# renmengye/rec-attend-public

Hardware: AMD Instinct MI355X
Metric: instance-timesteps/sec, full_model forward 512x512 T=16 (whole job; pipelined throughput: 8 batches in flight per GPU, fill and drain of the pipeline inside the timed region; config.lone_batch_* = one sync-bracketed forward) (higher is better)
Workload: dtype f32; 1 GPU; cfg2: CVPPP-arch full_model eval forward, 512x512, T=16, B=8 per GPU, y_out+s_out; arch=cvppp, H=512, W=512, T=16, batch_per_gpu=8, global_batch=8, parallelism=batch-sharded x1, no collective, ranks_in_communicator=1, hip_graph=True, tile_tickets=False, batches_in_flight=8, pipeline_slots=4, batches_per_launch=2, input=resident in HBM, output=left in HBM

## Files before the change

include/recattend.h:

```cpp
#ifndef RECATTEND_H_
#define RECATTEND_H_

#include <stddef.h>
#include <stdint.h>

#ifdef __cplusplus
extern "C" {
#endif

#define RA_E_INVALID (-1)
#define RA_E_SHAPE (-2)
#define RA_E_WORKSPACE (-3)
#define RA_E_HUNG_BFS (-12)
#define RA_E_HUNG_PATH (-13)
#define RA_E_HUNG_FLOW (-14)
#define RA_E_HUNG_EQUALIZE (-15)

#define RA_ABI_VERSION 114
int ra_version(void);
const char *ra_last_error_string(void);

int ra_debug_poison_lds(void *stream);
int ra_debug_park_xcd(int xcd, int n_wg, int lds_bytes, int millis, int *resident, void *stream);

// ... 227 lines not shown
int ra_extract_conv0_f32(const float *img, int Ci, int chan0, const float *canvas, int canvas_chan,
                         const float *attn_rec, int B, int H, int W, int Fh, int Fw, int use_gamma, float *patch,
                         const float *w0, const float *scale, const float *shift, int Cout, int relu, float *y0,
                         void *stream);
#define RA_PASTE_Y_PREFILLED 1
#define RA_PASTE_CANVAS_FLOORED 2
int ra_paste_direct_f32(const float *patch, int Cp, int pc, const float *attn, int B, int H, int W,
                        int Fh, int Fw, float beta, int disable_overwrite, float *canvas, float *img,
                        int Ci, int canvas_chan, float *y_out, size_t y_stride_b, int flags,
                        void *stream);
int ra_paste_score_direct_f32(const float *patch, int Cp, int pc, const float *attn, int B, int H,
                              int W, int Fh, int Fw, float beta, int disable_overwrite,
                              float *canvas, float *y_out, size_t y_stride_b, int flags,
                              const float *h, int K0, const float *core, int K1, const float *w,
                              const float *bias, float *s_out, size_t s_stride_b, void *stream);

#define RA_RESAMPLE_READ 0
#define RA_RESAMPLE_WRITE 1
#define RA_RESAMPLE_BOX 2
int ra_ctrl_train_supported(int G, int Cf, int hid, int iters, int nout);
size_t ra_ctrl_train_save_floats(int G, int Cf, int hid, int iters);
int ra_ctrl_train_fwd_f32(int B, int G, int Cf, int hid, int iters, int nout, const float *feat, const float *Wg,
                          const float *bg, const float *W0, const float *b0, const float *W1, const float *b1,
                          const float *Wc, const float *bc, float *h_last, float *co, float *save, void *stream);
int ra_ctrl_train_bwd_f32(int B, int G, int Cf, int hid, int iters, int nout, const float *feat, const float *Wg,
                          const float *W0, const float *W1, const float *Wc, const float *save, const float *dh_last,
                          const float *dco, float *dfeat, float *dpre, float *dz1, float *dlog, void *stream);
int ra_ctrl_train_supported_n(int G, int Cf, int hid, int iters, int nout, int n_glimpse, int n_ctrl, int mlp_dim);
size_t ra_ctrl_train_save_floats_n(int G, int Cf, int hid, int iters, int n_glimpse);
int ra_ctrl_train_fwd_n_f32(int B, int G, int Cf, int hid, int iters, int nout, int n_glimpse, int n_ctrl, int mlp_dim,
// ... 12 lines not shown
                        int Fw, const float *scale, int scale_stride, const float *div, int div_stride, float *ws,
                        size_t ws_floats, float *out, void *stream);
int ra_attn_box_direct_f32(const float *attn, int B, int H, int W, int Fh, int Fw, float beta,
                           float *box_out, size_t stride_b, void *stream);

int ra_extract_patch_dense_f32(const float *x, const float *f_y, const float *f_x, int B, int H,
                               int W, int D, int FH, int FW, float *out, void *stream);

int ra_dense_f32(const float *x0, int K0, const float *x1, int K1, const float *W, const float *b,
                 int B, int N, int act, float *out, size_t out_stride_b, void *stream);

int ra_pack_input_f32(const float *x, int D, const float *d_in, int Dd, const float *y_in, int Dy,
                      int B, int H, int W, int Cp, float *packed, void *stream);
int ra_pack_input_plane_f32(const float *x, int D, const float *d_in, int Dd, const float *y_in, int Dy,
                            int B, int H, int W, int Cp, float *packed, float *canvas_plane, void *stream);
int ra_canvas_max_f32(float *img, int Ci, int canvas_chan, const float *ysel, const float *noise,
                      int B, int H, int W, void *stream);

int ra_affine_act_f32(const float *x, const float *scale, const float *shift, size_t npix, int C,
                      int relu, float *y, void *stream);
int ra_max_pool_f32(const float *x, int B, int H, int W, int C, int ratio, float *y, void *stream);

enum {
  RA_STAT_LOSS = 0, RA_STAT_BOX_LOSS, RA_STAT_SEGM_LOSS, RA_STAT_CONF_LOSS, RA_STAT_IOU_SOFT,
  RA_STAT_IOU_SOFT_BOX, RA_STAT_WT_COV_SOFT, RA_STAT_UNWT_COV_SOFT, RA_STAT_IOU_HARD,
  RA_STAT_WT_COV_HARD, RA_STAT_UNWT_COV_HARD, RA_STAT_DICE, RA_STAT_COUNT_ACC, RA_STAT_DIC,
  RA_STAT_DIC_ABS, RA_STAT_COUNT
};
size_t ra_pair_stats_workspace_floats(int B, int HW);
int ra_pair_stats_f32(const float *a, const float *b, int B, int N, int M, int HW, float *ws,
// ... 320 lines not shown
```

rec-attend-public_amd/csrc/ra_attn.hip:

```cpp
#include "ra_common.h"

namespace ra {
namespace attn {

typedef float f32x4 __attribute__((ext_vector_type(4)));

__device__ inline float tap_mu(float ctr, float size, int F, int j) {
  return ctr + (size + 1.0f) / (float)F * ((float)j - ((float)F - 1.0f) / 2.0f);
}
__device__ inline float gauss(float l, float mu, float var) {
  const float d = l - mu;
  return (1.0f / sqrtf(var) / sqrtf(2.0f * 3.14159265358979323846f)) * expf(-0.5f * d * d / var);
}

__global__ void gaussian_filter_kernel(const float *center, const float *size, const float *lg_var,
                                       int B, int L, int F, float *out) {
  const size_t n = (size_t)B * L * F;
  for (size_t e = blockIdx.x * (size_t)blockDim.x + threadIdx.x; e < n;
       e += (size_t)gridDim.x * blockDim.x) {
    const int f = e % F;
    const int l = (e / F) % L;
    const int b = e / ((size_t)F * L);
    out[e] = gauss((float)l, tap_mu(center[b], size[b], F, f), expf(lg_var[b]));
  }
// ... 25 lines not shown
      __syncthreads();
      if (o < nout) {
        int wlo = (c0 - d + D - 1) / D;
        if (wlo < 0) wlo = 0;
        for (int w = wlo; w < W; ++w) {
          const int idx = w * D + d - c0;
          if (idx >= cn) break;
          acc += tbuf[idx] * fxb[(size_t)w * FW + fw];
        }
      }
    }
    if (o < nout) out[(((size_t)b * FH + fh) * FW + fw) * D + d] = acc;
  }
}

__global__ void pack_input_kernel(const float *x, int D, const float *d_in, int Dd, const float *y_in,
                                  int Dy, size_t npix, int Cp, float *packed, float *plane) {
  const int C4 = Cp >> 2;
  const size_t n = npix * C4;
  typedef float f32x4p __attribute__((ext_vector_type(4)));
  for (size_t e = blockIdx.x * (size_t)blockDim.x + threadIdx.x; e < n; e += (size_t)gridDim.x * blockDim.x) {
    const size_t p = e / C4;
    const int q = (int)(e - p * C4);
    if (plane && q == 0) plane[p] = 0.0f;
    f32x4p v;
#pragma unroll
    for (int j = 0; j < 4; ++j) {
      const int c = 4 * q + j;
      float val = 0.0f;
      if (c < D) val = x[p * D + c];
      else if (c > D && c <= D + Dd) val = d_in[p * Dd + (c - D - 1)];
      else if (c > D + Dd && c <= D + Dd + Dy) val = y_in[p * Dy + (c - D - 1 - Dd)];
      v[j] = val;
    }
    reinterpret_cast<f32x4p *>(packed)[e] = v;
  }
}

__global__ void canvas_max_kernel(float *img, int Ci, int canvas_chan, const float *ysel,
                                  const float *noise, size_t npix) {
  for (size_t p = blockIdx.x * (size_t)blockDim.x + threadIdx.x; p < npix;
       p += (size_t)gridDim.x * blockDim.x) {
    float v = ysel[p];
    if (noise) v = v - v * noise[p];
    float *c = img + p * Ci + canvas_chan;
    *c = fmaxf(v, *c);
  }
}

__global__ void affine_act_kernel(const float *x, const float *scale, const float *shift, size_t n,
// ... 63 lines not shown
}

extern "C" int ra_pack_input_plane_f32(const float *x, int D, const float *d_in, int Dd, const float *y_in,
                                       int Dy, int B, int H, int W, int Cp, float *packed, float *canvas_plane,
                                       void *stream) {
  if (!x || !packed || B <= 0 || H <= 0 || W <= 0 || D <= 0 || (Dd > 0 && !d_in) || (Dy > 0 && !y_in))
    return fail(RA_E_INVALID, "ra_pack_input_f32: bad argument");
  if (Cp % 4 || D + 1 + Dd + Dy > Cp || (reinterpret_cast<uintptr_t>(packed) & 15))
    return fail(RA_E_SHAPE, "ra_pack_input_f32: Cp %d (a multiple of 4 holding D + 1 + Dd + Dy channels), packed 16-byte aligned", Cp);
  const size_t npix = (size_t)B * H * W;
  hipLaunchKernelGGL(attn::pack_input_kernel, dim3(attn::grid_for(npix * (size_t)(Cp / 4), 256)), dim3(256), 0,
                     as_stream(stream), x, D, d_in, Dd, y_in, Dy, npix, Cp, packed, canvas_plane);
  return launch_status("ra_pack_input_f32");
}

extern "C" int ra_canvas_max_f32(float *img, int Ci, int canvas_chan, const float *ysel,
                                 const float *noise, int B, int H, int W, void *stream) {
  if (!img || !ysel || B <= 0 || H <= 0 || W <= 0 || canvas_chan < 0 || canvas_chan >= Ci)
    return fail(RA_E_INVALID, "ra_canvas_max_f32: bad argument");
  const size_t npix = (size_t)B * H * W;
  hipLaunchKernelGGL(attn::canvas_max_kernel, dim3(attn::grid_for(npix, 256)), dim3(256), 0,
                     as_stream(stream), img, Ci, canvas_chan, ysel, noise, npix);
  return launch_status("ra_canvas_max_f32");
}

extern "C" int ra_affine_act_f32(const float *x, const float *scale, const float *shift, size_t npix,
                                 int C, int relu, float *y, void *stream) {
  if (!x || !scale || !shift || !y || C <= 0) return fail(RA_E_INVALID, "ra_affine_act_f32: bad argument");
  if (npix == 0) return 0;
  const size_t n = npix * C;
// ... 16 lines not shown
```

rec-attend-public_amd/csrc/ra_attn_axis.h:

```cpp
#pragma once
#include "ra_common.h"

namespace ra {
namespace attnd {

typedef float f32x4 __attribute__((ext_vector_type(4)));
constexpr float kBandLog = 30.0f;
constexpr float kInvSqrt2Pi = 0.3989422804014327f;

struct Axis {
  float ctr, step, inv_step, half, inv2var, norm, R;
  int L, F;
  __device__ inline float mu(int j) const { return ctr + step * ((float)j - half); }
  __device__ inline float w(float l, int j) const {
    const float d = l - mu(j);
    return norm * __expf(-d * d * inv2var);
  }
  __device__ inline void band(int j, int &lo, int &hi) const {
    const float m = mu(j);
    float a = ceilf(m - R), c = floorf(m + R) + 1.0f;
    a = fminf(fmaxf(a, 0.0f), (float)L);
    c = fminf(fmaxf(c, 0.0f), (float)L);
    if (!(a == a) || !(c == c)) {
      a = 0.0f;
// ... 31 lines not shown
__device__ inline Axis make_axis(const float *rec, int axis, int L, int F) {
  Axis A;
  const float var = __expf(rec[4 + axis]);
  A.ctr = rec[0 + axis];
  A.step = (rec[2 + axis] + 1.0f) / (float)F;
  A.inv_step = __builtin_amdgcn_rcpf(A.step);
  A.half = ((float)F - 1.0f) / 2.0f;
  A.inv2var = 0.5f * __builtin_amdgcn_rcpf(var);
  A.norm = kInvSqrt2Pi * __builtin_amdgcn_rsqf(var);
  A.R = __builtin_amdgcn_sqrtf(2.0f * kBandLog * var);
  A.L = L;
  A.F = F;
  return A;
}

__device__ inline float readlane_f(float v, int l) {
  return __builtin_bit_cast(float, __builtin_amdgcn_readlane(__builtin_bit_cast(int, v), l));
}

}
}
```

rec-attend-public_amd/csrc/ra_attn_direct.hip:

```cpp
#include <cstdlib>

#include "ra_attn_parts.h"
#include "ra_common.h"

namespace ra {
namespace attnd {

#ifdef RA_PROBE
__device__ long long *ra_probe_buf;
#define RA_PROBE_AT(k)                                                                              \
  do {                                                                                              \
    if (threadIdx.x == 0)                                                                           \
      ra_probe_buf[(size_t)(blockIdx.x + gridDim.x * (blockIdx.y + gridDim.y * blockIdx.z)) * 8 + (k)] = wall_clock64(); \
  } while (0)
#else
#define RA_PROBE_AT(k)
#endif

struct Conv0Args {
  const float *w, *scale, *shift;
  int Cout, relu;
  float *y0;
};

// ... 481 lines not shown
    }
#pragma unroll
    for (int r = 0; r < RB; ++r) {
      if (!((live_mask >> r) & 1)) continue;
      const float cv = (MODE == 0) ? Cs[r * W + w] : 0.0f;
      float v = fast_sigmoid(acc[r] + beta);
      v -= dis * v * cv;
      __builtin_amdgcn_raw_buffer_store_b32(__builtin_bit_cast(unsigned, v), rsY, w * 4, r * W * 4, 0);
      if (MODE == 0)
        __builtin_amdgcn_raw_buffer_store_b32(__builtin_bit_cast(unsigned, fmaxf(cv, v)), rsV, w * 4, r * W * 4, 0);
    }
  }
  RA_PROBE_AT(4);
}

}
}

using namespace ra;

namespace {
struct PastePlan {
  int kernel, rows, grid_x, threads;
  size_t lds;
};
PastePlan choose_paste(int mode, int H, int W, int Fh, int Fw, int Cp, int pc, bool has_canvas, bool has_img, size_t y_stride_b,
                       bool aligned16, attnd::PasteGeo pg) {
  const int rb = pg.rows == 8 ? 8 : 4;
  const bool win_ok = W % 4 == 0 && Fw <= 64 && rb * W <= 4096 && (y_stride_b & 3) == 0 && aligned16 &&
                      (size_t)H * W * 4 < 0x7fffffffu && Fh * Fw % 4 == 0 && Fh * Fw <= 4 * attnd::kPsQuads * 256 &&
// ... 101 lines not shown
}

extern "C" int ra_paste_score_direct_f32(const float *patch, int Cp, int pc, const float *attn_rec, int B, int H,
                                         int W, int Fh, int Fw, float beta, int disable_overwrite, float *canvas,
                                         float *y_out, size_t y_stride_b, int flags, const float *h, int K0,
                                         const float *core, int K1, const float *w, const float *bias,
                                         float *s_out, size_t s_stride_b, void *stream) {
  if (!patch || !attn_rec || !y_out || !canvas || !h || !w || !s_out || B <= 0 || H <= 0 || W <= 0 || Fh <= 0 ||
      Fw <= 0 || Cp <= 0 || pc < 0 || pc >= Cp || K0 <= 0 || K1 < 0 || (K1 > 0 && !core))
    return fail(RA_E_INVALID, "ra_paste_score_direct_f32: bad argument");
  attnd::ScoreArgs sc{h, core, w, bias, s_out, K0, K1, s_stride_b};
  launch_paste<0>(1, patch, Cp, pc, attn_rec, B, H, W, Fh, Fw, beta, disable_overwrite, canvas, nullptr, 0, -1, y_out,
                  y_stride_b, disable_overwrite ? (flags & ~RA_PASTE_Y_PREFILLED) : flags, sc, stream);
  return launch_status("ra_paste_score_direct_f32");
}
```

rec-attend-public_amd/full_model.py:

```python
import os
import numpy as np
import torch

import modellib
import nnlib as nn
import ra_engine
import ra_ops as ops
from ra_native import RecAttendError


def _get(opt, key, default):
  return opt[key] if key in opt else default


def derive_dims(opt, box_model=False):
  d = {'T': opt['timespan'], 'H': opt['inp_height'], 'W': opt['inp_width'],
       'D': opt['inp_depth'], 'Fh': opt['filter_height'], 'Fw': opt['filter_width']}
  if d['H'] % 4 or d['W'] % 4:
    raise RecAttendError('inp_height / inp_width must be multiples of 4')
  if 'add_d_out' in opt:
    add_d, add_y = bool(opt['add_d_out']), bool(opt['add_y_out'])
  else:
    add_d = add_y = False
  assert (add_d and add_y) or (not add_d and not add_y)
# ... 308 lines not shown
    self.co_resident = int(co_resident or self.streams)
    self.coalesce = int(coalesce)
    self.slots = None
    self.free = list(range(self.depth))
    self.group = []
    self.pending = []

  def _make_slots(self):
    proto = self.model.engine
    self.slots = []
    prios = [int(v) for v in os.environ.get('RA_PIPE_PRIO', '').split(',') if v.strip()]
    streams = [torch.cuda.Stream(priority=prios[k % len(prios)]) if prios else torch.cuda.Stream() for k in range(self.streams)]
    for k in range(self.depth):
      eng = ra_engine.DecodeEngine(proto.d, self.model, box_model=proto.box)
      for flag in ('fuse_pairs', 'fuse_patch_pairs', 'ctrl_split', 'fuse_score',
                   'cache_first', 'fill_cache_inline', 'nsub', 'use_graph', 'use_wino', 'wino_unfuse', 'pair_wino', 'pair_direct16', 'prefill_ride',
                   'fuse_extract_conv0', 'use_split', 'split_first', 'split_patch', 'box_iou_rects', 'ctrl_batch_xcd'):
        setattr(eng, flag, getattr(proto, flag))
      eng.co_resident = self.co_resident
      eng.xcd_slot, eng.xcd_slots = k % self.streams, (self.streams if self.co_resident <= self.streams else 0)
      self.slots.append((eng, streams[k % self.streams]))

  def __len__(self):
    return len(self.pending)

  def parts(self, B):
    return 1 if not self.max_images else max(1, -(-int(B) // int(self.max_images)))

  def _ends_soon(self, remaining):
    return (remaining is not None and self.coalesce > 1 and len(self.group) + 1 + int(remaining) <= self.depth and
            os.environ.get('RA_PIPE_ENDGAME', '0') == '1')
# ... 32 lines not shown
    t = dict(names=names, single=single, feed=feed, to_host=to_host, B=B, launch=None, lo=0, hi=B)
    self.group.append(t)
    self.pending.append(t)
    if len(self.group) >= self.coalesce or ends:
      self._launch_group()

  def _launch_group(self):
    if not self.group:
      return
    members, self.group = self.group, []
    if self.slots is None:
      self._make_slots()
    names, to_host = members[0]['names'], members[0]['to_host']
    feeds = [m['feed'] for m in members]
    as_dev = lambda v: v if isinstance(v, torch.Tensor) else torch.from_numpy(np.ascontiguousarray(v, dtype=np.float32))
    if len(members) == 1:
      feed = feeds[0]
    else:
      feed = {}
      for k in ('x', 'd_in', 'y_in', 'y_gt'):
        if feeds[0].get(k) is not None:
          feed[k] = torch.cat([as_dev(f[k]).to('cuda', non_blocking=True) for f in feeds], dim=0)
      if feeds[0].get('noise') is not None:
        feed['noise'] = torch.cat([as_dev(f['noise']).to('cuda') for f in feeds], dim=1)
    B = sum(m['B'] for m in members)
    nparts = self.parts(B)
    if nparts > len(self.free):
      raise RecAttendError('%d of %d slots busy: collect() a batch before the next submit()' %
                           (self.depth - len(self.free), self.depth))
    bounds = [(B * i) // nparts for i in range(nparts + 1)]
    cut = lambda v, lo, hi: None if v is None else v[lo:hi]
    used, events = [], []
    for lo, hi in zip(bounds[:-1], bounds[1:]):
      k = self.free.pop(0)
      eng, stream = self.slots[k]
      stream.wait_stream(torch.cuda.current_stream())
      noise = feed.get('noise')
      with torch.cuda.stream(stream):
        eng.forward(cut(feed['x'], lo, hi), d_in=cut(feed.get('d_in'), lo, hi), y_in=cut(feed.get('y_in'), lo, hi),
                    y_gt=cut(feed.get('y_gt'), lo, hi) if self.model.box_model else None,
                    noise=None if noise is None else noise[:, lo:hi], want_box='attn_box' in names)
        host = None
        if to_host:
          host = []
          for n in names:
            r = self.model._fetch(n, eng)
# ... 192 lines not shown
```

rec-attend-public_amd/ra_engine.py:

```python
import numpy as np
import math
import os

import torch

import operator

import ra_native as rn
import ra_ops as ops


def _dev(a, device):
  return torch.from_numpy(np.ascontiguousarray(a)).to(device)


def _r4(n):
  return -(-n // 4) * 4


_TENSOR_VERSION = operator.attrgetter('_version')


class DecodeEngine(object):

  def __init__(self, dims, model, box_model=False):
    self.d = dims
    self.model = model
    self.box = box_model
    self._stamp = None
    self._B = None
    self._graphs = {}
    self.fuse_pairs = True
    self.fuse_patch_pairs = False
    self.ctrl_split = True
    self.fuse_score = True
    self.wino_unfuse = False
    self.pair_wino = True
    self.pair_direct16 = os.environ.get('RA_PAIR16', '1') != '0'
    self.use_wino = True
    self.cache_first = True
    self.fill_cache_inline = True
    self.co_resident = 1
    self.tile_tickets = os.environ.get('RA_ENGINE_TICKETS', '0') != '0'
    self.nsub = 0
    self.use_graph = True
    self.prefill_ride = True
    self.use_split = os.environ.get('RA_USE_SPLIT', '1') != '0'
    self.split_first = os.environ.get('RA_SPLIT_FIRST', '1') != '0'
    self.ctrl_batch_xcd = os.environ.get('RA_CTRL_BATCH_XCD', '1') != '0'
    self.xcd_slot, self.xcd_slots = 0, 1
    self.box_iou_rects = os.environ.get('RA_BOX_IOU_RECTS', '1') != '0'
    self.split_patch = os.environ.get('RA_SPLIT_PATCH', 'auto')
    self.fuse_extract_conv0 = os.environ.get('RA_FUSE_EXTRACT_CONV0', '0') == '1'
    self.timing = None

  def _weights_stamp(self):
    m = self.model
    mut = getattr(m, '_mut', None)
    if mut is None:
      return tuple((k, v.data_ptr(), v._version) for k, v in sorted(m.items())
                   if isinstance(v, torch.Tensor) and '_' in k and not k.startswith('__'))
# ... 212 lines not shown
    subs = []
    for k in range(nsub):
      b = {kk: v[k * Bs:(k + 1) * Bs] for kk, v in g.items() if kk != 'noise'}
      b['img'] = f(Bs, H, W, d['C0p'])
      b['canvas'] = f(Bs, H, W)
      hh, ww = H, W
      b['ccnn'] = []
      for i in range(d['ccnn_nlayers']):
        hh, ww = hh // d['ccnn_pool'][i], ww // d['ccnn_pool'][i]
        b['ccnn'].append(f(Bs, hh, ww, d['ccnn_channels'][i + 1]))
      b['tickets'] = ops.tickets_alloc(16 * T, device)
      b['h_last'] = f(T, Bs, d['hid'])
      b['ctrl_out'] = f(T, Bs, 9)
      b['gmaps'] = f(T, Bs, d['iters'], d['G'])
      b['attn'] = f(T, Bs, rn.RA_ATTN_STRIDE)
      st0 = self.plan['ccnn'][0]
      if self.cache_first and st0[0] == 'pair' and d['C0p'] == 4 and self.ksize['ccnn'][:2] == [3, 3] and \
          ops.first_cache_supported(4, d['ccnn_channels'][1], d['ccnn_channels'][2], d['ccnn_pool'][1], H, W):
        b['l0cache'] = ops.first_cache_alloc(Bs, H, W, device)
      form = ops.ctrl_form(self.desc, Bs, self.co_resident) if self.split_ok else None
      if form == 'split':
        b['ctrl_ws'], b['ctrl_status'] = ops.ctrl_split_workspace(self.desc, Bs, device)
      elif form == 'batch':
        b['ctrl_ws'], b['ctrl_status'] = ops.ctrl_batch_workspace(self.desc, Bs, device)
        b['ctrl_batch'] = True
        ng = -(-Bs // ops.ctrl_batch_group(self.desc, Bs))
        if self.ctrl_batch_xcd and self.xcd_slots >= 1 and self.xcd_slots * ng <= int(os.environ.get('RA_CTRL_BATCH_XCD_MAX_TEAMS', '4')):
          b['ctrl_xcd_off'] = (self.xcd_slot % self.xcd_slots) * ng
      if self.box:
        b['noise'] = f(T, Bs, H, W)
# ... 19 lines not shown
    self.glob = g
    self.subs = subs
    self.streams = [torch.cuda.Stream(device=device) for _ in range(nsub)] if nsub > 1 else []
    self._B = (B, nsub)
    self._graphs = {}

  def fetch(self, name):
    if name in self.glob:
      return self.glob[name]
    parts = [sb[name] for sb in self.subs]
    if len(parts) == 1:
      return parts[0]
    dim = 0 if name in ('img', 'canvas') else 1
    return torch.cat(parts, dim=dim)

  def check_status(self, recover=True):
    bad = False
    for sb in self.subs:
      st = sb.get('ctrl_status')
      if st is not None and int(st.item()) != 0:
        st.zero_()
        bad = True
    if not bad:
      return False
    if not recover:
      raise rn.RecAttendError('controller_split: a workgroup timed out waiting for its peers (the launch was '
                              'not fully resident); decode with engine.ctrl_split = False')
    import warnings
    warnings.warn('controller_split: a workgroup timed out waiting for its peers (the launch was not fully resident: is '
                  'something else using this GPU?); the batch is decoded again on the one-workgroup controller, which this '
                  'engine keeps from now on')
    torch.cuda.synchronize()
    keep = {k: self.glob[k].clone() for k in ('x', 'd_in', 'y_in', 'y_gt', 'noise') if k in self.glob}
    want_box = getattr(self, '_last_want_box', False)
    self.ctrl_split = False
    self._stamp = None
    self._B = None
    self._states = {}
    self._graphs = {}
    self.forward(keep['x'], d_in=keep.get('d_in'), y_in=keep.get('y_in'), y_gt=keep.get('y_gt'), noise=keep.get('noise'),
                 want_box=want_box)
    torch.cuda.synchronize()
    return True

  def _mark(self, name):
    if self.timing is not None:
      ev = torch.cuda.Event(enable_timing=True)
      ev.record()
      self.timing.append((name, ev))

  def stage_times_ms(self):
    out = {}
    for (_, e0), (name, e1) in zip(self.timing[:-1], self.timing[1:]):
      tot, n = out.get(name, (0.0, 0))
      out[name] = (tot + e0.elapsed_time(e1), n + 1)
    return out

# ... 3 lines not shown
      return
    main = torch.cuda.current_stream()
    for sb, st in zip(self.subs, self.streams):
      st.wait_stream(main)
      with torch.cuda.stream(st):
        self._launch_sub(sb, want_box)
    for st in self.streams:
      main.wait_stream(st)

  def _launch_sub(self, b, want_box):
    self._launch_pack(b)
    bound = self.tile_tickets and 'tickets' in b and ops.tickets_bind(b['tickets'])
    try:
      for tt in range(self.d['T']):
        self._launch_tail(b, tt, want_box, self._launch_encoder(b, tt))
    finally:
      if bound:
        ops.tickets_unbind()

  def _launch_encoder(self, b, tt):
    fill = b['y_out'] if (tt == 0 and b.pop('_fill_rider', False)) else None
    return self._run_cnn(self.plan['ccnn'], self.W['ccnn'], b['img'], b['ccnn'], tt, 'ctrl_cnn',
                         plane=b['canvas'], cache=b.get('l0cache'), fill=fill)

  def _prefill_rides(self, b):
    st0 = self.plan['ccnn'][0]
    return (self.prefill_ride and 'l0cache' in b and self.fill_cache_inline and st0[0] == 'pair' and
            ops.fill_rider_ok(b['y_out']))

  def _launch_pack(self, b):
    if self._prepacked:
      b['canvas'].zero_()
    else:
      ops.pack_input(b['x'], b.get('d_in'), b.get('y_in'), self.d['C0p'], b['img'],
                     canvas_plane=b['canvas'])
    if not self.box and not self.d['disable_overwrite']:
      if self._prefill_rides(b):
        b['_fill_rider'] = True
      else:
        ops.fill(b['y_out'], 1.0 / (1.0 + math.exp(5.0)))
    if 'l0cache' in b and not self.fill_cache_inline:
      ops.first_cache(b['img'], self.W['ccnn'][0][0], self.d['ccnn_channels'][1], self.d['D'], b['l0cache'])
    self._mark('pack')

  def _launch_tail(self, b, tt, want_box, src):
    d, Wt, T = self.d, self.W, self.d['T']
    H, W, Fh, Fw = d['H'], d['W'], d['Fh'], d['Fw']
    if 'ctrl_ws' in b and b.get('ctrl_batch'):
      ops.controller_batch(self.desc, src, Wt['ctrl_split'], b['h_last'][tt], b['ctrl_out'][tt], b['gmaps'][tt], b['attn'][tt],
                           b['ctrl_ws'], b['ctrl_status'], xcd_offset=b.get('ctrl_xcd_off', -1))
    elif 'ctrl_ws' in b:
      ops.controller_split(
# ... 111 lines not shown
    box = b['box1']
    if self.box_iou_rects and 'gt_params' in b and d['W'] % 4 == 0 and T <= 32:
      iou = ops.box_iou_rects(box.view(box.shape[0], d['H'], d['W']), b['gt_params'])
    else:
      iou = ops.pair_stats(box, b['box_gt'], want=('iou_soft',))['iou_soft']
    ops.greedy_match(iou.view(iou.shape[0], T), out=b['match'])
    ops.weighted_sum(b['match'], b['y_gt'], b['ysel'])
    ops.canvas_max(b['canvas'].view(b['canvas'].shape + (1,)), 0, b['ysel'], b['noise'][tt])
    nsc = d['nsc']
    ops.dense(b['h_last'][tt], self.W['smlp_w'], self.W['smlp_b'],
              'sigmoid' if nsc == 1 else 'softmax', b['s_out'].data_ptr() + tt * nsc * 4,
              T * nsc)
    self._mark('box_step')

  _prepacked = False

  def prestage_slots(self, B):
    if not torch.cuda.is_available():
      raise rn.RecAttendError('the decode loop needs an MI355X (HIP device); no CPU fallback')
    device = torch.device('cuda')
    if self._stamp is None:
      self.prepare(device)
    self.alloc(B, device)
    return self.subs

  def forward(self, x, d_in=None, y_in=None, y_gt=None, noise=None, want_box=False, prepacked=False):
    if not torch.cuda.is_available():
      raise rn.RecAttendError('the decode loop needs an MI355X (HIP device); no CPU fallback')
    self._prepacked = bool(prepacked)
    device = torch.device('cuda')
    as_t = lambda a: (a if isinstance(a, torch.Tensor) else torch.from_numpy(
        np.ascontiguousarray(a, dtype=np.float32))).to(device=device, dtype=torch.float32)
    x = as_t(x)
    B = x.shape[0]
    late_check = self._stamp is not None
    if not late_check:
      self.prepare(device)
    self.alloc(B, device)
    b = self.glob
    b['x'].copy_(x)
    if 'd_in' in b and not prepacked:
      b['d_in'].copy_(as_t(d_in))
    if 'y_in' in b and not prepacked:
      b['y_in'].copy_(as_t(y_in))
    if self.box:
      b['y_gt'].copy_(as_t(y_gt))
      if noise is None:
        b['noise'].uniform_(0.0, 0.3)
      else:
        b['noise'].copy_(as_t(noise).reshape(b['noise'].shape))
      Bs = B // len(self.subs)
      for k, sb in enumerate(self.subs):
        sb['noise'].copy_(b['noise'][:, k * Bs:(k + 1) * Bs])
        sb['gt_params'], sb['box_gt'] = ops.gt_box(sb['y_gt'].contiguous(), float(self.d['attn_box_padding_ratio']), 10.0)
    self._last_want_box = bool(want_box)
    self._launch_forward(want_box)
    if late_check and self._weights_stamp() != self._stamp:
      self.prepare(device)
      self._launch_forward(want_box)
    return self

  def _launch_forward(self, want_box):
    graphable = self.use_graph and self.timing is None
    if not graphable:
      self._launch_all(want_box)
      return self
    key = (bool(want_box), True) if self._prepacked else bool(want_box)
    if self.box:
      for sb in self.subs:
        if 'box_gt_buf' not in sb:
          sb['box_gt_buf'] = torch.empty_like(sb['box_gt'])
          sb['gt_params_buf'] = torch.empty_like(sb['gt_params'])
        sb['box_gt_buf'].copy_(sb['box_gt'])
        sb['box_gt'] = sb['box_gt_buf']
        sb['gt_params_buf'].copy_(sb['gt_params'])
        sb['gt_params'] = sb['gt_params_buf']
    g = self._graphs.get(key)
    if g is None:
      self._launch_all(want_box)
      torch.cuda.synchronize()
      g = torch.cuda.CUDAGraph()
      with rn.quiet_capture(), torch.cuda.graph(g):
        self._launch_all(want_box)
      self._graphs[key] = g
    g.replay()
    return self
```

rec-attend-public_amd/ra_ops.py:

```python
import ctypes as C
import os

import numpy as np
import torch

import ra_native as rn
from ra_native import check, ptr

BN_EPS = 1e-3


def _need_cuda(*ts, f32=True):
  for t in ts:
    if t is not None and not t.is_cuda:
      raise rn.RecAttendError('recattend kernels need CUDA (HIP) tensors; got a CPU tensor. '
                              'There is no CPU fallback.')
    if t is not None and ((f32 and t.dtype != torch.float32) or not t.is_contiguous()):
      raise rn.RecAttendError('recattend kernels need contiguous float32 tensors')


def _np32(a):
  if isinstance(a, torch.Tensor):
    a = a.detach().cpu().numpy()
  return np.ascontiguousarray(a, dtype=np.float32)
# ... 820 lines not shown
PASTE_Y_PREFILLED, PASTE_CANVAS_FLOORED = rn.RA_PASTE_Y_PREFILLED, rn.RA_PASTE_CANVAS_FLOORED


def paste_direct(patch, pc, attn, beta, disable_overwrite, y_out, y_stride_b, H, W, canvas=None,
                 img=None, canvas_chan=-1, flags=0):
  _need_cuda(patch, attn, canvas, img)
  B, Fh, Fw, Cp = patch.shape
  Ci = 0 if img is None else img.shape[3]
  check(rn.lib().ra_paste_direct_f32(ptr(patch), Cp, pc, ptr(attn), B, H, W, Fh, Fw, C.c_float(beta),
                                     int(disable_overwrite), ptr(canvas), ptr(img), Ci,
                                     int(canvas_chan), ptr(y_out), y_stride_b, int(flags),
                                     rn.stream_ptr()),
        'ra_paste_direct_f32')


def paste_score_direct(patch, pc, attn, beta, disable_overwrite, y_out, y_stride_b, H, W, canvas, flags,
                       h, core, w, bias, s_out_ptr, s_stride_b):
  _need_cuda(patch, attn, canvas, h, core, w, bias)
  B, Fh, Fw, Cp = patch.shape
  K1 = 0 if core is None else core.shape[1]
  check(rn.lib().ra_paste_score_direct_f32(ptr(patch), Cp, pc, ptr(attn), B, H, W, Fh, Fw, C.c_float(beta),
                                           int(disable_overwrite), ptr(canvas), ptr(y_out), y_stride_b,
                                           int(flags), ptr(h), h.shape[1], ptr(core), K1, ptr(w), ptr(bias),
                                           ptr(s_out_ptr), s_stride_b, rn.stream_ptr()),
        'ra_paste_score_direct_f32')


def paste_plan(mode, B, H, W, Fh, Fw, Cp=1, pc=0, has_canvas=True, has_img=False, y_stride_b=None, aligned16=True):
  rec = (C.c_int * rn.RA_PASTE_PLAN_INTS)()
  stride = H * W if y_stride_b is None else y_stride_b
# ... 39 lines not shown
  _need_cuda(x0, x1, W, b)
  code = {None: 0, 'relu': 1, 'sigmoid': 2, 'softmax': 3, 'tanh': 4}[act]
  K1 = 0 if x1 is None else x1.shape[1]
  check(rn.lib().ra_dense_f32(ptr(x0), x0.shape[1], ptr(x1), K1, ptr(W), ptr(b), x0.shape[0],
                              W.shape[1], code, ptr(out), out_stride_b, rn.stream_ptr()),
        'ra_dense_f32')


def pack_input(x, d_in, y_in, Cp, packed, canvas_plane=None):
  _need_cuda(x, d_in, y_in, packed, canvas_plane)
  B, H, W, D = x.shape
  Dd = 0 if d_in is None else d_in.shape[3]
  Dy = 0 if y_in is None else y_in.shape[3]
  check(rn.lib().ra_pack_input_plane_f32(ptr(x), D, ptr(d_in), Dd, ptr(y_in), Dy, B, H, W, Cp,
                                         ptr(packed), ptr(canvas_plane), rn.stream_ptr()), 'ra_pack_input_plane_f32')


def canvas_max(img, canvas_chan, ysel, noise):
  _need_cuda(img, ysel, noise)
  B, H, W, Ci = img.shape
  check(rn.lib().ra_canvas_max_f32(ptr(img), Ci, canvas_chan, ptr(ysel), ptr(noise), B, H, W,
                                   rn.stream_ptr()), 'ra_canvas_max_f32')


def gaussian_filter(center, size, lg_var, L, F):
  _need_cuda(center, size, lg_var)
  B = center.shape[0]
  out = torch.empty((B, L, F), dtype=torch.float32, device=center.device)
  check(rn.lib().ra_gaussian_filter_f32(ptr(center), ptr(size), ptr(lg_var), B, L, F, ptr(out),
                                        rn.stream_ptr()), 'ra_gaussian_filter_f32')
# ... 1025 lines not shown
```

Before: 61940 instance-timesteps/s.

## Pack inputs directly from per-batch sources and prefill only attention windows

Adds a multi-source pack kernel so per-batch feeds go straight into the packed image buffer, skipping the torch.cat and the staging copy into glob buffers. Also adds a fill_windows kernel that, once y_out is known clean from a prior run, refills only the rows and columns covered by each step's attention window rather than the whole y_out. A y_clean flag tracks validity and is reset on recovery. The cost is extra bookkeeping and a correctness risk if the flag becomes stale.

```diff
diff --git a/include/recattend.h b/include/recattend.h
--- a/include/recattend.h
+++ b/include/recattend.h
@@ -265,6 +265,8 @@
                               float *canvas, float *y_out, size_t y_stride_b, int flags,
                               const float *h, int K0, const float *core, int K1, const float *w,
                               const float *bias, float *s_out, size_t s_stride_b, void *stream);
+int ra_fill_windows_f32(float *y, size_t y_stride_b, int T, int B, int H, int W, int Fh, int Fw, const float *records,
+                        float value, const int *clean_flag, void *stream);
 
 #define RA_RESAMPLE_READ 0
 #define RA_RESAMPLE_WRITE 1
@@ -307,6 +309,9 @@
                       int B, int H, int W, int Cp, float *packed, void *stream);
 int ra_pack_input_plane_f32(const float *x, int D, const float *d_in, int Dd, const float *y_in, int Dy,
                             int B, int H, int W, int Cp, float *packed, float *canvas_plane, void *stream);
+int ra_pack_input_multi_f32(int nsrc, const float *const *x, const float *const *d_in, const float *const *y_in,
+                            const int *images, int D, int Dd, int Dy, int H, int W, int Cp, float *packed,
+                            float *canvas_plane, void *stream);
 int ra_canvas_max_f32(float *img, int Ci, int canvas_chan, const float *ysel, const float *noise,
                       int B, int H, int W, void *stream);
 
diff --git a/rec-attend-public_amd/csrc/ra_attn.hip b/rec-attend-public_amd/csrc/ra_attn.hip
--- a/rec-attend-public_amd/csrc/ra_attn.hip
+++ b/rec-attend-public_amd/csrc/ra_attn.hip
@@ -1,3 +1,6 @@
+#include <climits>
+#include <cstdint>
+
 #include "ra_common.h"
 
 namespace ra {
@@ -63,26 +66,57 @@
   }
 }
 
+__device__ __forceinline__ f32x4 pack_quad(const float *x, int D, const float *d_in, int Dd, const float *y_in, int Dy,
+                                            size_t p, int q) {
+  f32x4 v;
+#pragma unroll
+  for (int j = 0; j < 4; ++j) {
+    const int c = 4 * q + j;
+    float val = 0.0f;
+    if (c < D) val = x[p * D + c];
+    else if (c > D && c <= D + Dd) val = d_in[p * Dd + (c - D - 1)];
+    else if (c > D + Dd && c <= D + Dd + Dy) val = y_in[p * Dy + (c - D - 1 - Dd)];
+    v[j] = val;
+  }
+  return v;
+}
+
 __global__ void pack_input_kernel(const float *x, int D, const float *d_in, int Dd, const float *y_in,
                                   int Dy, size_t npix, int Cp, float *packed, float *plane) {
   const int C4 = Cp >> 2;
   const size_t n = npix * C4;
-  typedef float f32x4p __attribute__((ext_vector_type(4)));
   for (size_t e = blockIdx.x * (size_t)blockDim.x + threadIdx.x; e < n; e += (size_t)gridDim.x * blockDim.x) {
     const size_t p = e / C4;
     const int q = (int)(e - p * C4);
     if (plane && q == 0) plane[p] = 0.0f;
-    f32x4p v;
+    reinterpret_cast<f32x4 *>(packed)[e] = pack_quad(x, D, d_in, Dd, y_in, Dy, p, q);
+  }
+}
+
+constexpr int kPackSources = 8;
+struct PackSources {
+  const float *x[kPackSources], *d_in[kPackSources], *y_in[kPackSources];
+  size_t first[kPackSources];
+};
+
+__global__ void pack_input_multi_kernel(PackSources S, int D, int Dd, int Dy, size_t npix, int Cp, float *packed, float *plane) {
+  const int C4 = Cp >> 2;
+  const size_t n = npix * C4;
+  for (size_t e = blockIdx.x * (size_t)blockDim.x + threadIdx.x; e < n; e += (size_t)gridDim.x * blockDim.x) {
+    const size_t p = e / C4;
+    const int q = (int)(e - p * C4);
+    if (plane && q == 0) plane[p] = 0.0f;
+    const float *x = S.x[0], *d_in = S.d_in[0], *y_in = S.y_in[0];
+    size_t first = 0;
 #pragma unroll
-    for (int j = 0; j < 4; ++j) {
-      const int c = 4 * q + j;
-      float val = 0.0f;
-      if (c < D) val = x[p * D + c];
-      else if (c > D && c <= D + Dd) val = d_in[p * Dd + (c - D - 1)];
-      else if (c > D + Dd && c <= D + Dd + Dy) val = y_in[p * Dy + (c - D - 1 - Dd)];
-      v[j] = val;
+    for (int s = 1; s < kPackSources; ++s) {
+      const bool in = p >= S.first[s];
+      x = in ? S.x[s] : x;
+      d_in = in ? S.d_in[s] : d_in;
+      y_in = in ? S.y_in[s] : y_in;
+      first = in ? S.first[s] : first;
     }
-    reinterpret_cast<f32x4p *>(packed)[e] = v;
+    reinterpret_cast<f32x4 *>(packed)[e] = pack_quad(x, D, d_in, Dd, y_in, Dy, p - first, q);
   }
 }
 
@@ -176,6 +210,35 @@
   return launch_status("ra_pack_input_f32");
 }
 
+extern "C" int ra_pack_input_multi_f32(int nsrc, const float *const *x, const float *const *d_in, const float *const *y_in,
+                                       const int *images, int D, int Dd, int Dy, int H, int W, int Cp, float *packed,
+                                       float *canvas_plane, void *stream) {
+  if (nsrc < 1 || nsrc > attn::kPackSources || !x || !images || !packed || H <= 0 || W <= 0 || D <= 0 || Dd < 0 || Dy < 0 ||
+      (Dd > 0 && !d_in) || (Dy > 0 && !y_in))
+    return fail(RA_E_INVALID, "ra_pack_input_multi_f32: bad argument (1 .. %d sources)", attn::kPackSources);
+  attn::PackSources S;
+  const size_t hw = (size_t)H * W;
+  size_t B = 0;
+  for (int s = 0; s < attn::kPackSources; ++s) {
+    const bool live = s < nsrc;
+    S.x[s] = live ? x[s] : nullptr;
+    S.d_in[s] = live && d_in ? d_in[s] : nullptr;
+    S.y_in[s] = live && y_in ? y_in[s] : nullptr;
+    S.first[s] = live ? B * hw : SIZE_MAX;
+    if (!live) continue;
+    if (!x[s] || images[s] <= 0 || (S.d_in[s] != nullptr) != (S.d_in[0] != nullptr) || (S.y_in[s] != nullptr) != (S.y_in[0] != nullptr) ||
+        (Dd > 0 && !S.d_in[s]) || (Dy > 0 && !S.y_in[s]))
+      return fail(RA_E_INVALID, "ra_pack_input_multi_f32: source %d: x, d_in (all sources or none), y_in (likewise), images > 0", s);
+    B += (size_t)images[s];
+  }
+  if (Cp % 4 || D + 1 + Dd + Dy > Cp || (reinterpret_cast<uintptr_t>(packed) & 15) || B > (size_t)INT_MAX)
+    return fail(RA_E_SHAPE, "ra_pack_input_multi_f32: Cp %d (a multiple of 4 holding D + 1 + Dd + Dy channels), packed 16-byte aligned", Cp);
+  const size_t npix = B * hw;
+  hipLaunchKernelGGL(attn::pack_input_multi_kernel, dim3(attn::grid_for(npix * (size_t)(Cp / 4), 256)), dim3(256), 0,
+                     as_stream(stream), S, D, Dd, Dy, npix, Cp, packed, canvas_plane);
+  return launch_status("ra_pack_input_multi_f32");
+}
+
 extern "C" int ra_canvas_max_f32(float *img, int Ci, int canvas_chan, const float *ysel,
                                  const float *noise, int B, int H, int W, void *stream) {
   if (!img || !ysel || B <= 0 || H <= 0 || W <= 0 || canvas_chan < 0 || canvas_chan >= Ci)
diff --git a/rec-attend-public_amd/csrc/ra_attn_axis.h b/rec-attend-public_amd/csrc/ra_attn_axis.h
--- a/rec-attend-public_amd/csrc/ra_attn_axis.h
+++ b/rec-attend-public_amd/csrc/ra_attn_axis.h
@@ -69,6 +69,23 @@
   return A;
 }
 
+struct PasteWindow {
+  Axis Ay;
+  int wbeg, wend;
+  __device__ inline bool row(int l) const {
+    int jlo, jhi;
+    Ay.taps(l, jlo, jhi);
+    return jlo < jhi;
+  }
+};
+
+__device__ inline PasteWindow paste_window(const float *rec, int H, int W, int Fh, int Fw) {
+  PasteWindow p;
+  p.Ay = make_axis(rec, 0, H, Fh);
+  make_axis(rec, 1, W, Fw).span4(p.wbeg, p.wend);
+  return p;
+}
+
 __device__ inline float readlane_f(float v, int l) {
   return __builtin_bit_cast(float, __builtin_amdgcn_readlane(__builtin_bit_cast(int, v), l));
 }
diff --git a/rec-attend-public_amd/csrc/ra_attn_direct.hip b/rec-attend-public_amd/csrc/ra_attn_direct.hip
--- a/rec-attend-public_amd/csrc/ra_attn_direct.hip
+++ b/rec-attend-public_amd/csrc/ra_attn_direct.hip
@@ -519,6 +519,30 @@
   RA_PROBE_AT(4);
 }
 
+constexpr int kFillRows = 64;
+__global__ __launch_bounds__(256) void fill_windows_kernel(float *__restrict__ y, size_t y_stride_b, int T, int B, int H, int W,
+                                                            int Fh, int Fw, const float *__restrict__ records, float value,
+                                                            const int *__restrict__ clean, int vec, int chunks) {
+  const int lane = threadIdx.x & 63, wv = __builtin_amdgcn_readfirstlane(threadIdx.x >> 6);
+  const int plane = blockIdx.x / chunks, chunk = blockIdx.x - plane * chunks;
+  const int b = plane / T, t = plane - b * T;
+  const bool whole = *clean == 0;
+  const PasteWindow pw = paste_window(records + ((size_t)t * B + b) * RA_ATTN_STRIDE, H, W, Fh, Fw);
+  const int wbeg = whole ? 0 : pw.wbeg, wend = whole ? W : pw.wend;
+  const f32x4 v4 = f32x4{value, value, value, value};
+  const int l1 = (chunk + 1) * kFillRows < H ? (chunk + 1) * kFillRows : H;
+  float *base = y + (size_t)b * y_stride_b + (size_t)t * H * W;
+  for (int l = chunk * kFillRows + wv; l < l1; l += 4) {
+    if (!whole && !pw.row(l)) continue;
+    float *row = base + (size_t)l * W;
+    if (vec) {
+      for (int w = wbeg + 4 * lane; w < wend; w += 256) *reinterpret_cast<f32x4 *>(row + w) = v4;
+    } else {
+      for (int w = wbeg + lane; w < wend; w += 64) row[w] = value;
+    }
+  }
+}
+
 }
 }
 
@@ -650,3 +674,16 @@
                   y_stride_b, disable_overwrite ? (flags & ~RA_PASTE_Y_PREFILLED) : flags, sc, stream);
   return launch_status("ra_paste_score_direct_f32");
 }
+
+extern "C" int ra_fill_windows_f32(float *y, size_t y_stride_b, int T, int B, int H, int W, int Fh, int Fw, const float *records,
+                                   float value, const int *clean_flag, void *stream) {
+  if (!y || !records || !clean_flag || T <= 0 || B <= 0 || H <= 0 || W <= 0 || Fh <= 0 || Fw <= 0)
+    return fail(RA_E_INVALID, "ra_fill_windows_f32: bad argument");
+  if (y_stride_b < (size_t)T * H * W) return fail(RA_E_SHAPE, "ra_fill_windows_f32: image stride %zu < T H W", y_stride_b);
+  const int vec = W % 4 == 0 && (reinterpret_cast<uintptr_t>(y) & 15) == 0 && (y_stride_b & 3) == 0;
+  const int chunks = ceil_div(H, attnd::kFillRows);
+  if ((size_t)B * T * chunks > 0x7fffffffu) return fail(RA_E_SHAPE, "ra_fill_windows_f32: B T ceil(H / %d) exceeds 2^31", attnd::kFillRows);
+  hipLaunchKernelGGL(attnd::fill_windows_kernel, dim3((unsigned)((size_t)B * T * chunks)), dim3(256), 0, as_stream(stream), y, y_stride_b, T,
+                     B, H, W, Fh, Fw, records, value, clean_flag, vec, chunks);
+  return launch_status("ra_fill_windows_f32");
+}
diff --git a/rec-attend-public_amd/full_model.py b/rec-attend-public_amd/full_model.py
--- a/rec-attend-public_amd/full_model.py
+++ b/rec-attend-public_amd/full_model.py
@@ -346,7 +346,7 @@
     for k in range(self.depth):
       eng = ra_engine.DecodeEngine(proto.d, self.model, box_model=proto.box)
       for flag in ('fuse_pairs', 'fuse_patch_pairs', 'ctrl_split', 'fuse_score',
-                   'cache_first', 'fill_cache_inline', 'nsub', 'use_graph', 'use_wino', 'wino_unfuse', 'pair_wino', 'pair_direct16', 'prefill_ride',
+                   'cache_first', 'fill_cache_inline', 'nsub', 'use_graph', 'use_wino', 'wino_unfuse', 'pair_wino', 'pair_direct16', 'prefill_ride', 'pack_direct', 'prefill_windows',
                    'fuse_extract_conv0', 'use_split', 'split_first', 'split_patch', 'box_iou_rects', 'ctrl_batch_xcd'):
         setattr(eng, flag, getattr(proto, flag))
       eng.co_resident = self.co_resident
@@ -409,13 +409,17 @@
     names, to_host = members[0]['names'], members[0]['to_host']
     feeds = [m['feed'] for m in members]
     as_dev = lambda v: v if isinstance(v, torch.Tensor) else torch.from_numpy(np.ascontiguousarray(v, dtype=np.float32))
-    if len(members) == 1:
+    direct = self.slots[0][0].pack_direct
+    packed_keys = ('x', 'd_in', 'y_in') if direct else ()
+    if len(members) == 1 and not direct:
       feed = feeds[0]
     else:
       feed = {}
       for k in ('x', 'd_in', 'y_in', 'y_gt'):
-        if feeds[0].get(k) is not None:
-          feed[k] = torch.cat([as_dev(f[k]).to('cuda', non_blocking=True) for f in feeds], dim=0)
+        if feeds[0].get(k) is None:
+          continue
+        parts = [as_dev(f[k]).to(device='cuda', dtype=torch.float32, non_blocking=True).contiguous() for f in feeds]
+        feed[k] = parts if k in packed_keys else parts[0] if len(parts) == 1 else torch.cat(parts, dim=0)
       if feeds[0].get('noise') is not None:
         feed['noise'] = torch.cat([as_dev(f['noise']).to('cuda') for f in feeds], dim=1)
     B = sum(m['B'] for m in members)
@@ -424,7 +428,7 @@
       raise RecAttendError('%d of %d slots busy: collect() a batch before the next submit()' %
                            (self.depth - len(self.free), self.depth))
     bounds = [(B * i) // nparts for i in range(nparts + 1)]
-    cut = lambda v, lo, hi: None if v is None else v[lo:hi]
+    cut = lambda v, lo, hi: None if v is None else ra_engine._cut_batches(v, lo, hi) if isinstance(v, list) else v[lo:hi]
     used, events = [], []
     for lo, hi in zip(bounds[:-1], bounds[1:]):
       k = self.free.pop(0)
diff --git a/rec-attend-public_amd/ra_engine.py b/rec-attend-public_amd/ra_engine.py
--- a/rec-attend-public_amd/ra_engine.py
+++ b/rec-attend-public_amd/ra_engine.py
@@ -19,6 +19,16 @@
 
 
 _TENSOR_VERSION = operator.attrgetter('_version')
+
+
+def _cut_batches(batches, lo, hi):
+  out, first = [], 0
+  for t in batches:
+    a, b = max(lo, first), min(hi, first + t.shape[0])
+    if a < b:
+      out.append(t if (a, b) == (first, first + t.shape[0]) else t[a - first:b - first])
+    first += t.shape[0]
+  return out
 
 
 class DecodeEngine(object):
@@ -45,6 +55,8 @@
     self.nsub = 0
     self.use_graph = True
     self.prefill_ride = True
+    self.pack_direct = os.environ.get('RA_PACK_DIRECT', '1') != '0'
+    self.prefill_windows = os.environ.get('RA_PREFILL_WINDOWS', '1') != '0'
     self.use_split = os.environ.get('RA_USE_SPLIT', '1') != '0'
     self.split_first = os.environ.get('RA_SPLIT_FIRST', '1') != '0'
     self.ctrl_batch_xcd = os.environ.get('RA_CTRL_BATCH_XCD', '1') != '0'
@@ -287,6 +299,8 @@
       b['ctrl_out'] = f(T, Bs, 9)
       b['gmaps'] = f(T, Bs, d['iters'], d['G'])
       b['attn'] = f(T, Bs, rn.RA_ATTN_STRIDE)
+      if not self.box:
+        b['y_clean'] = torch.zeros((1,), dtype=torch.int32, device=device)
       st0 = self.plan['ccnn'][0]
       if self.cache_first and st0[0] == 'pair' and d['C0p'] == 4 and self.ksize['ccnn'][:2] == [3, 3] and \
           ops.first_cache_supported(4, d['ccnn_channels'][1], d['ccnn_channels'][2], d['ccnn_pool'][1], H, W):
@@ -336,6 +350,12 @@
     dim = 0 if name in ('img', 'canvas') else 1
     return torch.cat(parts, dim=dim)
 
+  def invalidate_outputs(self):
+    for subs in [self.__dict__.get('subs') or []] + [st[1] for st in self.__dict__.get('_states', {}).values()]:
+      for sb in subs:
+        if 'y_clean' in sb:
+          sb['y_clean'].zero_()
+
   def check_status(self, recover=True):
     bad = False
     for sb in self.subs:
@@ -343,8 +363,11 @@
       if st is not None and int(st.item()) != 0:
         st.zero_()
         bad = True
+    feeds = self._feeds
     if not bad:
+      self._feeds = None
       return False
+    self.invalidate_outputs()
     if not recover:
       raise rn.RecAttendError('controller_split: a workgroup timed out waiting for its peers (the launch was '
                               'not fully resident); decode with engine.ctrl_split = False')
@@ -360,9 +383,12 @@
     self._B = None
     self._states = {}
     self._graphs = {}
+    if feeds is not None:
+      keep['x'], keep['d_in'], keep['y_in'] = feeds
     self.forward(keep['x'], d_in=keep.get('d_in'), y_in=keep.get('y_in'), y_gt=keep.get('y_gt'), noise=keep.get('noise'),
                  want_box=want_box)
     torch.cuda.synchronize()
+    self._feeds = None
     return True
 
   def _mark(self, name):
@@ -396,6 +422,8 @@
     try:
       for tt in range(self.d['T']):
         self._launch_tail(b, tt, want_box, self._launch_encoder(b, tt))
+      if 'y_clean' in b and self.prefill_windows and self.timing is None and not self.d['disable_overwrite']:
+        ops.fill(b['y_clean'].view(torch.float32), 1.0)
     finally:
       if bound:
         ops.tickets_unbind()
@@ -407,17 +435,25 @@
 
   def _prefill_rides(self, b):
     st0 = self.plan['ccnn'][0]
+    if self.prefill_windows and 'y_clean' in b:
+      return False
     return (self.prefill_ride and 'l0cache' in b and self.fill_cache_inline and st0[0] == 'pair' and
             ops.fill_rider_ok(b['y_out']))
 
   def _launch_pack(self, b):
-    if self._prepacked:
+    if self._direct:
+      pass
+    elif self._prepacked:
       b['canvas'].zero_()
     else:
       ops.pack_input(b['x'], b.get('d_in'), b.get('y_in'), self.d['C0p'], b['img'],
                      canvas_plane=b['canvas'])
     if not self.box and not self.d['disable_overwrite']:
-      if self._prefill_rides(b):
+      if self.prefill_windows and 'y_clean' in b:
+        if self.timing is not None:
+          b['y_clean'].zero_()
+        ops.fill_windows(b['y_out'], b['attn'], self.d['Fh'], self.d['Fw'], 1.0 / (1.0 + math.exp(5.0)), b['y_clean'])
+      elif self._prefill_rides(b):
         b['_fill_rider'] = True
       else:
         ops.fill(b['y_out'], 1.0 / (1.0 + math.exp(5.0)))
@@ -559,6 +595,7 @@
     self._mark('box_step')
 
   _prepacked = False
+  _direct, _feeds = False, None
 
   def prestage_slots(self, B):
     if not torch.cuda.is_available():
@@ -569,6 +606,21 @@
     self.alloc(B, device)
     return self.subs
 
+  def _pack_feeds(self):
+    xs, d_ins, y_ins = self._feeds
+    Bs = self._B[0] // len(self.subs)
+    cut = lambda group, lo, hi: None if group is None else _cut_batches(group, lo, hi)
+    for k, sb in enumerate(self.subs):
+      lo = k * Bs
+      sx, sd, sy = cut(xs, lo, lo + Bs), cut(d_ins, lo, lo + Bs), cut(y_ins, lo, lo + Bs)
+      off = 0
+      for c in range(0, len(sx), ops.PACK_MULTI_SOURCES):
+        part = slice(c, c + ops.PACK_MULTI_SOURCES)
+        n = sum(t.shape[0] for t in sx[part])
+        ops.pack_input_multi(sx[part], None if sd is None else sd[part], None if sy is None else sy[part], self.d['C0p'],
+                             sb['img'][off:off + n], canvas_plane=sb['canvas'][off:off + n])
+        off += n
+
   def forward(self, x, d_in=None, y_in=None, y_gt=None, noise=None, want_box=False, prepacked=False):
     if not torch.cuda.is_available():
       raise rn.RecAttendError('the decode loop needs an MI355X (HIP device); no CPU fallback')
@@ -576,18 +628,32 @@
     device = torch.device('cuda')
     as_t = lambda a: (a if isinstance(a, torch.Tensor) else torch.from_numpy(
         np.ascontiguousarray(a, dtype=np.float32))).to(device=device, dtype=torch.float32)
-    x = as_t(x)
-    B = x.shape[0]
+    self._direct, self._feeds = False, None
+    if isinstance(x, (list, tuple)):
+      as_list = lambda group: None if group is None else [as_t(t).contiguous() for t in group]
+      feeds = (as_list(x), as_list(d_in) if self.d['add_d_out'] else None, as_list(y_in) if self.d['add_y_out'] else None)
+      for name, group, fed in (('d_in', feeds[1], self.d['add_d_out']), ('y_in', feeds[2], self.d['add_y_out'])):
+        if fed and (group is None or len(group) != len(feeds[0])) and not prepacked:
+          raise rn.RecAttendError('forward: the model reads %s: one per batch of x' % name)
+      if self.pack_direct and not prepacked:
+        self._direct, self._feeds = True, feeds
+        B = sum(t.shape[0] for t in feeds[0])
+      else:
+        x, d_in, y_in = (None if group is None else torch.cat(group, dim=0) for group in feeds)
+    if not self._direct:
+      x = as_t(x)
+      B = x.shape[0]
     late_check = self._stamp is not None
     if not late_check:
       self.prepare(device)
     self.alloc(B, device)
     b = self.glob
-    b['x'].copy_(x)
-    if 'd_in' in b and not prepacked:
-      b['d_in'].copy_(as_t(d_in))
-    if 'y_in' in b and not prepacked:
-      b['y_in'].copy_(as_t(y_in))
+    if not self._direct:
+      b['x'].copy_(x)
+      if 'd_in' in b and not prepacked:
+        b['d_in'].copy_(as_t(d_in))
+      if 'y_in' in b and not prepacked:
+        b['y_in'].copy_(as_t(y_in))
     if self.box:
       b['y_gt'].copy_(as_t(y_gt))
       if noise is None:
@@ -607,10 +673,12 @@
 
   def _launch_forward(self, want_box):
     graphable = self.use_graph and self.timing is None
+    if self._direct:
+      self._pack_feeds()
     if not graphable:
       self._launch_all(want_box)
       return self
-    key = (bool(want_box), True) if self._prepacked else bool(want_box)
+    key = (bool(want_box), 'direct') if self._direct else (bool(want_box), True) if self._prepacked else bool(want_box)
     if self.box:
       for sb in self.subs:
         if 'box_gt_buf' not in sb:
@@ -628,5 +696,7 @@
       with rn.quiet_capture(), torch.cuda.graph(g):
         self._launch_all(want_box)
       self._graphs[key] = g
+      if self._direct:
+        self._pack_feeds()
     g.replay()
     return self
diff --git a/rec-attend-public_amd/ra_ops.py b/rec-attend-public_amd/ra_ops.py
--- a/rec-attend-public_amd/ra_ops.py
+++ b/rec-attend-public_amd/ra_ops.py
@@ -858,6 +858,17 @@
         'ra_paste_direct_f32')
 
 
+def fill_windows(y, records, Fh, Fw, value, clean_flag):
+  _need_cuda(records, clean_flag, f32=False)
+  B, T, H, W = y.shape
+  if (not y.is_cuda or y.dtype != torch.float32 or y.stride()[1:] != (H * W, W, 1) or tuple(records.shape) != (T, B, rn.RA_ATTN_STRIDE) or
+      records.dtype != torch.float32 or clean_flag.element_size() != 4):
+    raise rn.RecAttendError('fill_windows: y float32 [B,T,H,W] with dense planes, records float32 [T,B,%d]' % rn.RA_ATTN_STRIDE)
+  check(rn.lib().ra_fill_windows_f32(ptr(y), y.stride(0), T, B, H, W, Fh, Fw, ptr(records), C.c_float(value), ptr(clean_flag),
+                                     rn.stream_ptr()), 'ra_fill_windows_f32')
+  return y
+
+
 def paste_score_direct(patch, pc, attn, beta, disable_overwrite, y_out, y_stride_b, H, W, canvas, flags,
                        h, core, w, bias, s_out_ptr, s_stride_b):
   _need_cuda(patch, attn, canvas, h, core, w, bias)
@@ -927,6 +938,35 @@
   Dy = 0 if y_in is None else y_in.shape[3]
   check(rn.lib().ra_pack_input_plane_f32(ptr(x), D, ptr(d_in), Dd, ptr(y_in), Dy, B, H, W, Cp,
                                          ptr(packed), ptr(canvas_plane), rn.stream_ptr()), 'ra_pack_input_plane_f32')
+
+
+PACK_MULTI_SOURCES = 8
+
+
+def pack_input_multi(xs, d_ins, y_ins, Cp, packed, canvas_plane=None):
+  n = len(xs)
+  _need_cuda(packed, canvas_plane, *xs)
+  for group in (d_ins, y_ins):
+    if group is not None:
+      _need_cuda(*group)
+  _, H, W, D = xs[0].shape
+  for k, group in enumerate((xs, d_ins, y_ins)):
+    if group is None:
+      continue
+    if len(group) != n:
+      raise rn.RecAttendError('pack_input_multi: %d x but %d %s' % (n, len(group), ('x', 'd_in', 'y_in')[k]))
+    chans = set(t.shape[3] for t in group if t is not None)
+    for t, x in zip(group, xs):
+      if t is not None and (t.dim() != 4 or tuple(t.shape[:3]) != (x.shape[0], H, W) or len(chans) != 1):
+        raise rn.RecAttendError('pack_input_multi: every source is a contiguous float32 [B_s, %d, %d, C]' % (H, W))
+  first = lambda group: None if group is None else group[0]
+  Dd = 0 if first(d_ins) is None else d_ins[0].shape[3]
+  Dy = 0 if first(y_ins) is None else y_ins[0].shape[3]
+  if sum(x.shape[0] for x in xs) != packed.shape[0]:
+    raise rn.RecAttendError('pack_input_multi: packed holds %d images, the sources %d' % (packed.shape[0], sum(x.shape[0] for x in xs)))
+  arr = lambda group: None if group is None else (C.c_void_p * n)(*[ptr(t) for t in group])
+  check(rn.lib().ra_pack_input_multi_f32(n, arr(xs), arr(d_ins), arr(y_ins), (C.c_int * n)(*[x.shape[0] for x in xs]), D, Dd, Dy,
+                                         H, W, Cp, ptr(packed), ptr(canvas_plane), rn.stream_ptr()), 'ra_pack_input_multi_f32')
 
 
 def canvas_max(img, canvas_chan, ysel, noise):
```

New measurement: 61910 instance-timesteps/s, median of 2. About the same (-0.1%).
